# djeedai/bevy_hanabi

Measured on AMD Instinct MI355X. Metric: particle-updates/sec, higher is better.
Workload: dtype f32

## Files before the change

### bevy_hanabi_amd/csrc/hnb_kernels.hip.h

```cpp
#pragma once
#ifndef __HIPCC_RTC__
#include <hip/hip_runtime.h>
#endif
#include "hnb_dev.h"

namespace hnb {

template <class T>
__device__ __forceinline__ T* global_ptr(uint64_t addr) {
    typedef __attribute__((address_space(1))) T global_t;
    return (T*)(global_t*)addr;
}

struct u2_t { uint32_t x, y; };
struct u3_t { uint32_t x, y, z; };
typedef uint32_t u4v __attribute__((ext_vector_type(4)));
#if defined(HNB_NONTEMPORAL) || defined(HNB_NONTEMPORAL_LOADS)
#define HNB_NT_LOAD(p) __builtin_nontemporal_load(p)
#else
#define HNB_NT_LOAD(p) (*(p))
#endif
#if defined(HNB_NONTEMPORAL) || defined(HNB_NONTEMPORAL_STORES)
#define HNB_NT_STORE(v, p) __builtin_nontemporal_store(v, p)
#else
#define HNB_NT_STORE(v, p) (*(p) = (v))
#endif

template <class T> __device__ __forceinline__ T ld_hint(const T* p, bool nt) { return nt ? __builtin_nontemporal_load(p) : *p; }
template <class T> __device__ __forceinline__ void st_hint(T v, T* p, bool nt) { if (nt) __builtin_nontemporal_store(v, p); else *p = v; }

__device__ __forceinline__ void lds_barrier() { asm volatile("s_waitcnt lgkmcnt(0)\n\ts_barrier" ::: "memory"); }

#define HNB_DPP_(v, ident, ctrl, rows) ((uint32_t)__builtin_amdgcn_update_dpp((int)(ident), (int)(v), ctrl, rows, 0xf, false))
#define HNB_WAVE_STEP_(v, ident, OP, ctrl, rows) { const uint32_t t_ = HNB_DPP_(v, ident, ctrl, rows); v = OP(v, t_); }
#define HNB_WAVE_REDUCE_(v, ident, OP)                                                          \
    HNB_WAVE_STEP_(v, ident, OP, 0xB1, 0xf)                            \
    HNB_WAVE_STEP_(v, ident, OP, 0x4E, 0xf)                            \
    HNB_WAVE_STEP_(v, ident, OP, 0x124, 0xf)                                     \
    HNB_WAVE_STEP_(v, ident, OP, 0x128, 0xf)   \
    HNB_WAVE_STEP_(v, ident, OP, 0x142, 0xa)                \
    HNB_WAVE_STEP_(v, ident, OP, 0x143, 0xc)
__device__ __forceinline__ uint32_t wave_sum_u32(uint32_t v) {
#define HNB_OP_(a, b) ((a) + (b))
    HNB_WAVE_REDUCE_(v, 0u, HNB_OP_)
#undef HNB_OP_
    return (uint32_t)__builtin_amdgcn_readlane((int)v, 63);
}
__device__ __forceinline__ uint32_t wave_min_u32(uint32_t v) {
#define HNB_OP_(a, b) ((b) < (a) ? (b) : (a))
    HNB_WAVE_REDUCE_(v, 0xffffffffu, HNB_OP_)
#undef HNB_OP_
    return (uint32_t)__builtin_amdgcn_readlane((int)v, 63);
}
__device__ __forceinline__ uint32_t wave_max_u32(uint32_t v) {
#define HNB_OP_(a, b) ((b) > (a) ? (b) : (a))
    HNB_WAVE_REDUCE_(v, 0u, HNB_OP_)
#undef HNB_OP_
    return (uint32_t)__builtin_amdgcn_readlane((int)v, 63);
}
__device__ __forceinline__ float wave_min_f32(float x) {
    uint32_t v = f2u(x);
#define HNB_OP_(a, b) f2u(fminf(u2f(a), u2f(b)))
    HNB_WAVE_REDUCE_(v, 0x7f800000u, HNB_OP_)
#undef HNB_OP_
    return u2f((uint32_t)__builtin_amdgcn_readlane((int)v, 63));
}


#ifndef HNB_JIT_TU
__global__ void k_reset_lists(uint32_t* __restrict__ dead, uint32_t* __restrict__ alive0, uint32_t* __restrict__ alive1, uint32_t capacity) {
    uint32_t i = blockIdx.x * blockDim.x + threadIdx.x;
    if (i < capacity) { dead[i] = i; alive0[i] = 0u; alive1[i] = 0u; }
}
#endif

#ifndef HNB_JIT_TU
struct ProbeArgs { uint32_t n_planes; uint32_t stride16[8]; uint64_t off[8]; uint32_t write_mask; uint32_t salt; uint64_t n_quads; };
__global__ void __launch_bounds__(256) k_probe_placement(char* __restrict__ base, const ProbeArgs a) {
    const uint64_t q = (uint64_t)blockIdx.x * 256u + threadIdx.x;
    if (q >= a.n_quads) return;
    uint32_t acc = 0;
#pragma unroll
    for (uint32_t pl = 0; pl < 8; ++pl) {
        if (pl >= a.n_planes) break;
        uint4* ptr = reinterpret_cast<uint4*>(base + a.off[pl]) + q * a.stride16[pl];
        for (uint32_t i = 0; i < a.stride16[pl]; ++i) {
            uint4 v = ptr[i];
            acc += v.x + v.y + v.z + v.w;
            v.x ^= a.salt;
            if (a.write_mask >> pl & 1u) ptr[i] = v;
        }
    }
    if (acc == 0x9e3779b9u && a.salt) *reinterpret_cast<uint32_t*>(base) = acc;
}
#endif

template <class FILE_T>
__device__ __forceinline__ void vfile_store_attr(const FILE_T& r, uint32_t ncomp, uint32_t reg, char* plane, uint32_t slot) {
    switch (ncomp) {
        case 1: reinterpret_cast<uint32_t*>(plane)[slot] = r[reg]; break;
        case 2: reinterpret_cast<u2_t*>(plane)[slot] = u2_t{r[reg], r[reg + 1]}; break;
        case 3: reinterpret_cast<u3_t*>(plane)[slot] = u3_t{r[reg], r[reg + 1], r[reg + 2]}; break;
        default: reinterpret_cast<uint4*>(plane)[slot] = make_uint4(r[reg], r[reg + 1], r[reg + 2], r[reg + 3]); break;
    }
}
__device__ __forceinline__ Out4 vfile_load_attr(uint32_t ncomp, const char* plane, uint32_t slot) {
    Out4 o = Out4{0u, 0u, 0u, 0u};
    switch (ncomp) {
        case 1: o.v0 = reinterpret_cast<const uint32_t*>(plane)[slot]; break;
        case 2: { const u2_t t = reinterpret_cast<const u2_t*>(plane)[slot]; o.v0 = t.x; o.v1 = t.y; } break;
        case 3: { const u3_t t = reinterpret_cast<const u3_t*>(plane)[slot]; o.v0 = t.x; o.v1 = t.y; o.v2 = t.z; } break;
        default: { const uint4 t = reinterpret_cast<const uint4*>(plane)[slot]; o.v0 = t.x; o.v1 = t.y; o.v2 = t.z; o.v3 = t.w; } break;
    }
    return o;
}

__device__ __forceinline__ void pin_scalar(uint32_t v) { asm volatile("" ::"s"(v)); }
__device__ __forceinline__ uint32_t requested_spawn(const DevFrameInst& f) {
    const uint4 h0 = reinterpret_cast<const uint4*>(&f)[0], h1 = reinterpret_cast<const uint4*>(&f)[1];
    const uint32_t spawn_count = h0.x, parity = h1.z, skip = h1.w;
    const uint64_t ev_in = (uint64_t)h1.x | ((uint64_t)h1.y << 32);
    pin_scalar(spawn_count);
    if (skip) return 0u;
    if (ev_in == 0ull) return spawn_count;
    const DevEventBuffer* ev = global_ptr<const DevEventBuffer>(ev_in);
    const uint2 cnt = *reinterpret_cast<const uint2*>(ev->count);
    const uint32_t n = (parity ^ 1u) ? cnt.y : cnt.x, cap = ev->capacity;
    return n < cap ? n : cap;
}

struct InterpCode {
    using file_t = vreg_file_t;
    template <class ST>
    static __device__ __forceinline__ void run_init(const DevProgram& p, ST& S, const VmUniforms& U, const VmAttrIO& io) {
        vm_run<true, false>(p.init_code, p.init_len, S, U, nullptr, nullptr, io);
    }
    template <class ST>
    static __device__ __forceinline__ void run_update(const DevProgram& p, ST& S, const VmUniforms& U, const VmAttrIO& io) {
        vm_run<true, false>(p.update_code, p.update_len, S, U, nullptr, nullptr, io);
    }
    static __device__ __forceinline__ void zero_unassigned(const DevProgram& p, const VmAttrIO& io) {
        for (uint32_t a = 0; a < p.n_attrs; ++a) {
            if (p.attrs[a].reg != HNB_REG_NONE) continue;
            uint32_t* q = vm_attr_ptr(io, a);
            for (uint32_t c = 0; c < p.attrs[a].ncomp; ++c) q[c] = 0u;
        }
    }
    template <class ST>
    static __device__ __forceinline__ void store_init(const DevProgram& p, const ST& S, char* base, uint32_t slot) {
        for (uint32_t a = 0; a < p.n_attrs; ++a)
            if (p.attrs[a].reg != HNB_REG_NONE) vfile_store_attr(S.r, p.attrs[a].ncomp, p.attrs[a].reg, base + p.attrs[a].plane_off, slot);
    }
    template <class ST>
    static __device__ __forceinline__ void load_update(const DevProgram& p, ST& S, const char* base, uint32_t slot, bool valid) {
        for (uint32_t a = 0; a < p.n_attrs; ++a) {
            const DevAttr at = p.attrs[a];
            if (!(at.upd_flags & HNB_ATTR_UPD_LOAD) || at.reg == HNB_REG_NONE) continue;
            Out4 o = Out4{0u, 0u, 0u, 0u};
            if (valid) o = vfile_load_attr(at.ncomp, base + at.plane_off, slot);
            for (uint32_t cc = 0; cc < at.ncomp; ++cc) S.r[at.reg + cc] = out4_get(o, cc);
        }
    }
    template <class ST>
    static __device__ __forceinline__ void store_update(const DevProgram& p, const ST& S, char* base, uint32_t slot) {
// ... 867 lines not shown




__device__ __forceinline__ void store_died_bits(uint32_t* __restrict__ bits, uint32_t step_first, uint32_t nib, uint32_t lane) {
    int v = (int)(nib << (4u * (lane & 7u)));
    v |= __builtin_amdgcn_update_dpp(0, v, 0xB1, 0xf, 0xf, true);
    v |= __builtin_amdgcn_update_dpp(0, v, 0x4E, 0xf, 0xf, true);
    v |= __builtin_amdgcn_update_dpp(0, v, 0x141, 0xf, 0xf, true);
    if ((lane & 7u) == 0u) bits[(step_first >> 5) + (lane >> 3)] = (uint32_t)v;
}

struct StreamLds {
    uint32_t died[kBlock / 64];
    float lmin[kBlock / 64];
    uint32_t alive[kBlock / 64];
    float rem[kBlock / 64];
    uint32_t amin[kBlock / 64], amax[kBlock / 64];
    u4v xp[2][kBlock / 64][kStepRows * 3u / 4u];
};
__device__ __forceinline__ StreamLds& stream_lds() {
    __shared__ StreamLds s;
    return s;
}

template <class PROG, int PROBE, bool COHORT, bool FUSED = false>
__device__ __forceinline__ void update_stream_chunk(const SlotArgs& args, const uint64_t* __restrict__ inst_base, const DevFrameInst* __restrict__ fi,
                                                    const uint32_t* __restrict__ ublocks, const CompactBufs& cb,
                                                    const uint32_t wg, const uint32_t wg_total) {
    StreamLds& lds = stream_lds();
    uint32_t (&s_died)[kBlock / 64] = lds.died;
    float (&s_lmin)[kBlock / 64] = lds.lmin;
    uint32_t (&s_alive)[kBlock / 64] = lds.alive;
    float (&s_rem)[kBlock / 64] = lds.rem;
    uint32_t (&s_amin)[kBlock / 64] = lds.amin;
    uint32_t (&s_amax)[kBlock / 64] = lds.amax;
    u4v (&s_xp)[2][kBlock / 64][kStepRows * 3u / 4u] = lds.xp;
    const uint32_t tid = threadIdx.x, lane = tid & 63u, wave = tid >> 6;
    const bool split = !FUSED && !COHORT && args.quarters == 4u;
    const uint32_t S = FUSED ? args.fuse_steps : 1u;
    const uint32_t chunk = split ? chunk_of_workgroup(cb.xcd_remap, wg >> 2, wg_total >> 2) : chunk_of_workgroup(cb.xcd_remap, wg, wg_total);
    const uint32_t quarter = split ? (wg & 3u) : 0u;
    const uint32_t k = chunk / args.chunks_per_inst, j = chunk - k * args.chunks_per_inst;
    const uint32_t wave0 = j * kChunk + (split ? (quarter * (kBlock / 64u) + wave) * kStepRows : wave * kWaveRows);
    const uint32_t n_steps = split ? 1u : kWaveRows / kStepRows;
    const uint32_t n_words = split ? wg_total >> 2 : wg_total;
    const uint32_t frozen = fi[k].skip;
    const uint64_t slab = inst_base[k];
    const bool store_nt = args.store_hint != 0u;
#ifndef HNB_PUBLISH_FIRST_WG
#define HNB_PUBLISH_FIRST_WG 1
#endif
    if (args.safe_words && (HNB_PUBLISH_FIRST_WG ? wg == 0u : chunk == 0u)) {
        uint32_t* prev = args.safe_words + (size_t)(args.safe_parity ^ 1u) * args.safe_stride;
        uint32_t m = 0x7f800000u;
        for (uint32_t i = tid; i < n_words; i += kBlock) { const uint32_t v = prev[i]; prev[i] = 0x7f800000u; m = v < m ? v : m; }
        m = wave_min_u32(m);
        if (lane == 0) s_alive[wave] = m;
        __syncthreads();
        if (tid == 0u) {
            for (uint32_t w = 1; w < kBlock / 64; ++w) m = s_alive[w] < m ? s_alive[w] : m;
            *reinterpret_cast<volatile unsigned long long*>(args.safe_host) = ((unsigned long long)m << 32) | (unsigned long long)args.publish_tag;
        }
        __syncthreads();
    }
    if (args.skip_lists && j == 0u && quarter == 0u && tid == 0u) {
        DevMeta o = args.meta_in[k];
        if constexpr (FUSED) {
            DevMeta before = o;
            if (!frozen) {
                o.max_update = o.alive_count; o.dead_count = 0u; o.spawned = 0u; o.instance_count = o.alive_count;
                before = o;
                o.ref_write_index ^= S & 1u;
                before.ref_write_index ^= (S - 1u) & 1u;
            }
            DevMeta* row_in = const_cast<DevMeta*>(args.meta_in);
            ((S & 1u) ? args.meta_out : row_in)[k] = o;
            ((S & 1u) ? row_in : args.meta_out)[k] = before;
            cb.deaths[(size_t)(cb.parity ^ 1u) * cb.table_cap + k] = 0u;
        } else {
        if (!frozen) {
            o.ref_write_index ^= 1u;
            o.max_update = o.alive_count; o.dead_count = 0u; o.spawned = 0u; o.instance_count = o.alive_count;
        }
        args.meta_out[k] = o;
        cb.deaths[(size_t)(cb.parity ^ 1u) * cb.table_cap + k] = 0u;
        }
    }
    if (frozen) return;
    char* base = global_ptr<char>(slab);
    VmUniforms U;
    U.u = ublocks + (size_t)k * args.n_uregs * S;
    auto uniforms_of = [&](const uint32_t s) { VmUniforms Us = U; Us.u = U.u + (size_t)s * args.n_uregs; return Us; };
    U.xf = fi[k].xf;
    float rem_min = __builtin_inff();
    char* p_pos = base + args.plane_off[0];
    char* p_vel = base + args.plane_off[1];
    char* p_age = base + args.plane_off[2];
    char* p_life = base + args.plane_off[3];
    uint32_t* flags4 = reinterpret_cast<uint32_t*>(base + args.alive_flag_off);
    const uint32_t fl = args.flags;
    uint32_t died_total = 0;
    uint32_t* cfull = reinterpret_cast<uint32_t*>(base + args.lmin_off) + args.chunks_per_inst;
    const bool chunk_full = cfull[j] == 1u;
    uint32_t* astate = cfull + args.chunks_per_inst;
    uint32_t* aval = astate + args.chunks_per_inst;
    const uint32_t ast_raw = COHORT ? astate[j] : 0u;
    bool check_due = ((args.frame_phase + j) & 15u) == 0u;
    if constexpr (FUSED) {
        for (uint32_t s = 1; s < S; ++s) check_due = check_due || ((args.frame_phase + s + j) & 15u) == 0u;
    }
    const bool mixed = COHORT && ast_raw == 4u && !check_due;
    const uint32_t ast = ast_raw == 4u ? 0u : ast_raw;
    const float A = COHORT ? u2f(aval[j]) : 0.0f;
    uint32_t amin = 0xffffffffu, amax = 0u;
    uint32_t lane_alive = 0;
    const bool cull = args.cull_lifetime != 0u;
    float* lmin = reinterpret_cast<float*>(base + args.lmin_off);
    const float Lm = cull ? lmin[j] : 0.0f;
    const float dt_tick = cull ? uf(U, args.dt_operand) : 0.0f;
    auto age_after = [&](float a) {
        if constexpr (FUSED) {
            for (uint32_t s = 0; s < S; ++s) a = a + uf(uniforms_of(s), args.dt_operand);
            return a;
        } else return a + dt_tick;
    };
    if (args.horizon && j == 0u && quarter == 0u && tid == 0u) {
        double* clk = horizon_view(base, args.horizon_off, args.chunks_per_inst).clock;
        if constexpr (FUSED) {
            double c = *clk;
            for (uint32_t s = 0; s < S; ++s) { const float t = cull ? uf(uniforms_of(s), args.dt_operand) : 0.0f; c = c + (double)(t > 0.0f ? t : 0.0f) * (1.0 + 0x1p-16); }
            *clk = c;
        } else
        *clk = *clk + (double)(dt_tick > 0.0f ? dt_tick : 0.0f) * (1.0 + 0x1p-16);
    }
    float wave_min = __builtin_inff();
    bool loaded_all = true;
    bool flat = false;
    if constexpr (PROG::kFlat && COHORT && PROBE == 0) {
        flat = chunk_full && ast == 1u && cull && Lm > 0.0f && (age_after(A) < Lm) && (fl & 3u) == 3u && !(fl & 128u);
    }
    if (flat) {
        if constexpr (PROG::kFlat && COHORT && PROBE == 0) {
            const float A2 = age_after(A);
            u4v* pw = reinterpret_cast<u4v*>(p_pos + (size_t)j * (kChunk * 12u)) + wave * (kWaveRows * 3u / 4u);
            u4v* vw = reinterpret_cast<u4v*>(p_vel + (size_t)j * (kChunk * 12u)) + wave * (kWaveRows * 3u / 4u);
            const uint32_t rot = lane % 3u;
            if (args.age_current && (fl & 64u)) {
                u4v* aw = reinterpret_cast<u4v*>(p_age + (size_t)j * (kChunk * 4u)) + wave * (kWaveRows / 4u);
                const uint32_t a2 = f2u(A2);
#pragma unroll
                for (uint32_t step = 0; step < kWaveRows / kStepRows; ++step) aw[step * 64u + lane] = u4v{a2, a2, a2, a2};
            }
#pragma unroll 2
            for (uint32_t step = 0; step < kWaveRows / kStepRows; ++step) {
                float P[3][4], V[3][4];
#pragma unroll
                for (uint32_t w = 0; w < 3; ++w) {
                    const u4v a = pw[(step * 3u + w) * 64u + lane], b = vw[(step * 3u + w) * 64u + lane];
                    P[w][0] = u2f(a.x); P[w][1] = u2f(a.y); P[w][2] = u2f(a.z); P[w][3] = u2f(a.w);
                    V[w][0] = u2f(b.x); V[w][1] = u2f(b.y); V[w][2] = u2f(b.z); V[w][3] = u2f(b.w);
                }
                if constexpr (FUSED) {
                    for (uint32_t s = 0; s < S; ++s) PROG::run_flat(args.update_code, P, V, rot, uniforms_of(s));
                } else
                PROG::run_flat(args.update_code, P, V, rot, U);
#pragma unroll
                for (uint32_t w = 0; w < 3; ++w) {
                    if (fl & 16u) pw[(step * 3u + w) * 64u + lane] = u4v{f2u(P[w][0]), f2u(P[w][1]), f2u(P[w][2]), f2u(P[w][3])};
                    if (fl & 32u) vw[(step * 3u + w) * 64u + lane] = u4v{f2u(V[w][0]), f2u(V[w][1]), f2u(V[w][2]), f2u(V[w][3])};
                }
            }
            if (args.write_died && lane < kWaveRows / 32u)
                reinterpret_cast<uint32_t*>(base + args.died_bits_off)[((j * kChunk + wave * kWaveRows) >> 5) + lane] = 0u;
            amin = amax = f2u(A2);
            loaded_all = false;
            if (args.safe_words) rem_min = (f2u(A2) >> 31) ? 0.0f : (Lm - A2) - 1.0e-5f * Lm;
        }
    }
    auto step_body = [&](auto coh_tag, const uint32_t step, const uint32_t f4, const u4v* pre_age = nullptr) {
        constexpr bool COH = decltype(coh_tag)::value;
        const uint32_t s0 = wave0 + step * kStepRows + lane * 4u;
        bool was[4], fresh[4];
#pragma unroll
        for (int p = 0; p < 4; ++p) {
            const uint32_t byte = (f4 >> (8 * p)) & 0xffu;
            fresh[p] = COH && byte == 3u;
            was[p] = byte == 1u || fresh[p];
            lane_alive += was[p] ? 1u : 0u;
        }
        const bool any = was[0] || was[1] || was[2] || was[3];
        if (!__any(any)) {
            if (args.write_died) store_died_bits(reinterpret_cast<uint32_t*>(base + args.died_bits_off), s0 - lane * 4u, 0u, lane);
            return;
        }
        const bool full = was[0] && was[1] && was[2] && was[3];
        uint32_t slot[4];
#pragma unroll
        for (int p = 0; p < 4; ++p) slot[p] = s0 + p;
        bool lanes_on[4] = {any, any, any, any};
        Pinned<4> X;
#pragma unroll
        for (int p = 0; p < 4; ++p) { X.pos[p] = V3{0, 0, 0}; X.vel[p] = V3{0, 0, 0}; X.age[p] = 0.0f; X.lifetime[p] = 0.0f; X.alive[p] = true; }
        bool need_life = true;
        float age_was[4] = {0.0f, 0.0f, 0.0f, 0.0f};
        const uint32_t step_first = s0 - lane * 4u;
        const bool xp = args.transpose != 0u && PROBE == 0 && step_first + kStepRows <= args.capacity && __popcll(__ballot(any)) >= 32;
        if (xp) {
            if (fl & 1u) xpose_load3(X.pos, p_pos, step_first, s_xp[0][wave], lane);
            if (fl & 2u) xpose_load3(X.vel, p_vel, step_first, s_xp[1][wave], lane);
        }
        if (any) {
            if (!xp) {
                if (fl & 1u) pin_load3<4>(X.pos, p_pos, slot, lanes_on, true);
                if (fl & 2u) pin_load3<4>(X.vel, p_vel, slot, lanes_on, true);
            }
            if (fl & 4u) {
                if (!COH || ast != 1u) {
                    if (pre_age) { X.age[0] = u2f(pre_age->x); X.age[1] = u2f(pre_age->y); X.age[2] = u2f(pre_age->z); X.age[3] = u2f(pre_age->w); }
                    else pin_load1<4>(X.age, p_age, slot, lanes_on, true);
                    for (int p = 0; p < 4; ++p) age_was[p] = X.age[p];
                }
                if (COH && ast != 0u) {
#pragma unroll
                    for (int p = 0; p < 4; ++p) X.age[p] = fresh[p] ? X.age[p] : A;
                }
            }
        }
        if (cull && Lm > 0.0f && (COH || !mixed)) {
            bool may_die = false;
#pragma unroll
            for (int p = 0; p < 4; ++p) may_die = may_die || (was[p] && !(age_after(X.age[p]) < Lm));
            need_life = __any(may_die);
        }
        if (any && (fl & 8u)) {
            if (need_life) {
                if (args.stream_hint) {
                    const u4v ql = __builtin_nontemporal_load(reinterpret_cast<const u4v*>(p_life) + (slot[0] >> 2));
                    X.lifetime[0] = u2f(ql.x); X.lifetime[1] = u2f(ql.y); X.lifetime[2] = u2f(ql.z); X.lifetime[3] = u2f(ql.w);
                } else pin_load1<4>(X.lifetime, p_life, slot, lanes_on, true);
            }
            else {
#pragma unroll
                for (int p = 0; p < 4; ++p) X.lifetime[p] = Lm;
            }
        }
        if (!need_life) loaded_all = false;
        if constexpr (FUSED) {
            bool gone[4] = {false, false, false, false};
            for (uint32_t s = 0; s < S; ++s) {
                PROG::template run<4>(args.update_code, args.update_len, X, uniforms_of(s));
#pragma unroll
                for (int p = 0; p < 4; ++p) gone[p] = gone[p] || !X.alive[p];
            }
#pragma unroll
            for (int p = 0; p < 4; ++p) X.alive[p] = !gone[p];
        } else
        if constexpr (!(PROBE & 8)) PROG::template run<4>(args.update_code, args.update_len, X, U);
        if constexpr (!(PROBE & 4)) {
            const bool xp_pos = xp && (fl & 17u) == 17u, xp_vel = xp && (fl & 34u) == 34u;
            if (xp_pos) xpose_store3(X.pos, p_pos, step_first, s_xp[0][wave], lane, was, full, store_nt);
            if (xp_vel) xpose_store3(X.vel, p_vel, step_first, s_xp[1][wave], lane, was, full, store_nt);
            if (any) {
                if ((fl & 16u) && !xp_pos) pin_store3<4>(X.pos, p_pos, slot, was, full);
                if ((fl & 32u) && !xp_vel) pin_store3<4>(X.vel, p_vel, slot, was, full);
                if (fl & 64u) {
                    const bool plane_loaded = !COH || ast != 1u;
                    if (plane_loaded || args.age_current) {
                        if (plane_loaded && (fl & 4u) && !full) {
                            float q[4];
#pragma unroll
                            for (int p = 0; p < 4; ++p) q[p] = was[p] ? X.age[p] : age_was[p];
                            pin_store1<4>(q, p_age, slot, was, true, store_nt);
                        } else pin_store1<4>(X.age, p_age, slot, was, full, store_nt);
                    }
                }
                if (fl & 128u) pin_store1<4>(X.lifetime, p_life, slot, was, full);
            }
        } else {
            float acc = 0.0f;
#pragma unroll
            for (int p = 0; p < 4; ++p) acc += X.pos[p].x + X.pos[p].y + X.pos[p].z + X.vel[p].x + X.vel[p].y + X.vel[p].z + X.age[p] + X.lifetime[p];
            if (acc == 123.456f) X.alive[0] = false;
        }
        if (cull && need_life) {
#pragma unroll
            for (int p = 0; p < 4; ++p)
                if (was[p] && X.alive[p]) wave_min = fminf(wave_min, X.lifetime[p]);
        }
        if (args.safe_words) {
#pragma unroll
            for (int p = 0; p < 4; ++p)
                if (was[p] && X.alive[p]) rem_min = fminf(rem_min, (f2u(X.age[p]) >> 31) ? 0.0f : (X.lifetime[p] - X.age[p]) - 1.0e-5f * X.lifetime[p]);
        }
        if constexpr (COH) {
#pragma unroll
            for (int p = 0; p < 4; ++p) {
                const bool stays = was[p] && X.alive[p];
                const uint32_t b = f2u(X.age[p]);
                amin = (stays && b < amin) ? b : amin;
                amax = (stays && b > amax) ? b : amax;
            }
            if constexpr (!(PROBE & 4)) {
                const bool dies = (was[0] && !X.alive[0]) || (was[1] && !X.alive[1]) || (was[2] && !X.alive[2]) || (was[3] && !X.alive[3]);
                if (ast == 1u && (fl & 64u) && !args.age_current && __any(dies)) {
#pragma unroll
                    for (int p = 0; p < 4; ++p)
                        if (was[p] && !X.alive[p]) reinterpret_cast<float*>(p_age)[slot[p]] = X.age[p];
                }
            }
        }
        uint32_t nf = f4, nib = 0u;
        uint32_t died_here = 0;
#pragma unroll
        for (int p = 0; p < 4; ++p) {
            const bool died = was[p] && !X.alive[p];
            if (died) { nf &= ~(0xffu << (8 * p)); nib |= 1u << p; }
            else if (COH && fresh[p]) nf = (nf & ~(0xffu << (8 * p))) | (1u << (8 * p));
            died_here += (uint32_t)__popcll(__ballot(died));
        }
        if (nf != f4) flags4[s0 >> 2] = nf;
        if (args.write_died) store_died_bits(reinterpret_cast<uint32_t*>(base + args.died_bits_off), step_first, nib, lane);
        died_total += died_here;
    };
    if (!flat) {
// ... 540 lines not shown
```

### bevy_hanabi_amd/csrc/hnb_vm.h

```cpp
#pragma once
#include "hnb_math.h"
#ifdef __HIPCC_RTC__
#include "hanabi_amd.h"
#else
#include "../../include/hanabi_amd.h"
#endif

namespace hnb {

struct __attribute__((aligned(8))) Ins { uint32_t x, y; };

#ifdef HNB_VM_BOUNDS_CHECK
extern "C" void hnb_vm_oob(uint32_t index, uint32_t size);
template <uint32_t N>
struct checked_file_t {
    uint32_t v[N];
    uint32_t& operator[](uint32_t i) { if (i >= N) hnb_vm_oob(i, N); return v[i < N ? i : 0]; }
    const uint32_t& operator[](uint32_t i) const { if (i >= N) hnb_vm_oob(i, N); return v[i < N ? i : 0]; }
};
typedef checked_file_t<HNB_VM_MAX_REGS> vreg_file_t;
typedef checked_file_t<HNB_VM_MAX_REGS_WIDE> vreg_file_wide_t;
typedef checked_file_t<HNB_VM_MAX_UREGS> UFile;
#else
typedef uint32_t vreg_file_t __attribute__((vector_size(HNB_VM_MAX_REGS * 4)));
// ... 660 lines not shown
                const V3 v = uf3(U, a);
#pragma unroll
                for (int p = 0; p < P; ++p) mac_vel_add(X.vel[p], v);
            } break;
            case HNB_OP_M_PIN_SET: {
                if (d == HNB_REG_POSITION || d == HNB_REG_VELOCITY) {
                    const V3 v = uf3(U, a);
#pragma unroll
                    for (int p = 0; p < P; ++p) { if (d == HNB_REG_POSITION) X.pos[p] = v; else X.vel[p] = v; }
                } else {
                    const float s = uf(U, a);
#pragma unroll
                    for (int p = 0; p < P; ++p) { if (d == HNB_REG_AGE) X.age[p] = s; else X.lifetime[p] = s; }
                }
            } break;
            case HNB_OP_M_RADIAL_ACCEL:
                if constexpr (FULL) {
                    const V3 origin = uf3(U, a);
                    const float s = uf(U, b);
#pragma unroll
                    for (int p = 0; p < P; ++p) mac_radial_accel(X.pos[p], X.vel[p], origin, s);
                }
                break;
            case HNB_OP_M_TANGENT_ACCEL:
                if constexpr (FULL) {
                    const V3 origin = uf3(U, a), axis = uf3(U, b);
                    const float s = uf(U, c);
#pragma unroll
                    for (int p = 0; p < P; ++p) mac_tangent_accel(X.pos[p], X.vel[p], origin, axis, s);
                }
                break;
            case HNB_OP_M_CONFORM_SPHERE:
                if constexpr (FULL) {
                    ConformParams q;
                    q.c = uf3(U, a);
                    q.radius = uf(U, a + 3); q.influence_dist = uf(U, a + 4); q.shell_half_thickness = uf(U, a + 5);
                    q.max_attraction_speed = uf(U, a + 6); q.attraction_accel = uf(U, a + 7); q.sticky_factor = uf(U, a + 8);
                    const float dt = uf(U, b);
#pragma unroll
                    for (int p = 0; p < P; ++p) mac_conform_sphere(X.pos[p], X.vel[p], q, dt);
                }
                break;
            case HNB_OP_M_KILL_SPHERE: {
                const V3 center = uf3(U, a);
                const float r2 = uf(U, b);
#pragma unroll
                for (int p = 0; p < P; ++p) mac_kill_sphere(X.pos[p], center, r2, (aux & 1u) != 0u, X.alive[p]);
            } break;
            case HNB_OP_M_KILL_AABB: {
                const V3 center = uf3(U, a), half = uf3(U, b);
#pragma unroll
                for (int p = 0; p < P; ++p) mac_kill_aabb(X.pos[p], center, half, (aux & 1u) != 0u, X.alive[p]);
            } break;
            default: break;
        }
    }
}


template <uint32_t OP, int P>
HNB_HD void apply_static(const Ins ins, Pinned<P>& X, const VmUniforms& U) {
    const uint32_t a = HNB_OPERAND_DECODE((ins.x >> 16) & 0xffu, ins.y >> 13), b = HNB_OPERAND_DECODE(ins.x >> 24, ins.y >> 14);
    const uint32_t c = HNB_OPERAND_DECODE(ins.y & 0xffu, ins.y >> 15), aux = ins.y >> 16;
    if constexpr (OP == HNB_OP_M_AGE_TICK) {
        const float dt = uf(U, a);
        const bool has_lifetime = (aux & 1u) != 0u;
#pragma unroll
        for (int p = 0; p < P; ++p) mac_age_tick(X.age[p], X.lifetime[p], dt, has_lifetime, X.alive[p]);
    } else if constexpr (OP == HNB_OP_M_EULER) {
        const float dt = uf(U, a);
#pragma unroll
        for (int p = 0; p < P; ++p) mac_euler(X.pos[p], X.vel[p], dt);
    } else if constexpr (OP == HNB_OP_M_VEL_SCALE) {
        const float s = uf(U, a);
#pragma unroll
        for (int p = 0; p < P; ++p) mac_vel_scale(X.vel[p], s);
    } else if constexpr (OP == HNB_OP_M_VEL_ADD) {
        const V3 v = uf3(U, a);
#pragma unroll
        for (int p = 0; p < P; ++p) mac_vel_add(X.vel[p], v);
    } else if constexpr (OP == HNB_OP_M_PIN_SET) {
        const uint32_t d = (ins.x >> 8) & 0xffu;
        if (d == HNB_REG_POSITION || d == HNB_REG_VELOCITY) {
            const V3 v = uf3(U, a);
#pragma unroll
            for (int p = 0; p < P; ++p) { if (d == HNB_REG_POSITION) X.pos[p] = v; else X.vel[p] = v; }
        } else {
            const float s = uf(U, a);
#pragma unroll
            for (int p = 0; p < P; ++p) { if (d == HNB_REG_AGE) X.age[p] = s; else X.lifetime[p] = s; }
        }
    } else if constexpr (OP == HNB_OP_M_RADIAL_ACCEL) {
        const V3 origin = uf3(U, a);
        const float s = uf(U, b);
#pragma unroll
        for (int p = 0; p < P; ++p) mac_radial_accel(X.pos[p], X.vel[p], origin, s);
    } else if constexpr (OP == HNB_OP_M_TANGENT_ACCEL) {
        const V3 origin = uf3(U, a), axis = uf3(U, b);
        const float s = uf(U, c);
#pragma unroll
        for (int p = 0; p < P; ++p) mac_tangent_accel(X.pos[p], X.vel[p], origin, axis, s);
    } else if constexpr (OP == HNB_OP_M_CONFORM_SPHERE) {
        ConformParams q;
        q.c = uf3(U, a);
        q.radius = uf(U, a + 3); q.influence_dist = uf(U, a + 4); q.shell_half_thickness = uf(U, a + 5);
        q.max_attraction_speed = uf(U, a + 6); q.attraction_accel = uf(U, a + 7); q.sticky_factor = uf(U, a + 8);
        const float dt = uf(U, b);
#pragma unroll
        for (int p = 0; p < P; ++p) mac_conform_sphere(X.pos[p], X.vel[p], q, dt);
    } else if constexpr (OP == HNB_OP_M_KILL_SPHERE) {
        const V3 center = uf3(U, a);
        const float r2 = uf(U, b);
        const bool inside = (aux & 1u) != 0u;
#pragma unroll
        for (int p = 0; p < P; ++p) mac_kill_sphere(X.pos[p], center, r2, inside, X.alive[p]);
    } else if constexpr (OP == HNB_OP_M_KILL_AABB) {
        const V3 center = uf3(U, a), half = uf3(U, b);
        const bool inside = (aux & 1u) != 0u;
#pragma unroll
        for (int p = 0; p < P; ++p) mac_kill_aabb(X.pos[p], center, half, inside, X.alive[p]);
    } else {
        static_assert(OP == HNB_OP_M_AGE_TICK, "apply_static: opcode is not a streamable macro op");
    }
}

HNB_HD float rot3(const V3 v, uint32_t c) { return c == 0u ? v.x : (c == 1u ? v.y : v.z); }
template <uint32_t OP>
HNB_HD void apply_static_flat(const Ins ins, float (&pos)[3][4], float (&vel)[3][4], uint32_t rot, const VmUniforms& U) {
    const uint32_t a = HNB_OPERAND_DECODE((ins.x >> 16) & 0xffu, ins.y >> 13);
    if constexpr (OP == HNB_OP_M_EULER) {
        const float dt = uf(U, a);
#pragma unroll
        for (int j = 0; j < 3; ++j)
#pragma unroll
            for (int e = 0; e < 4; ++e) pos[j][e] = pos[j][e] + vel[j][e] * dt;
    } else if constexpr (OP == HNB_OP_M_VEL_SCALE) {
        const float s = uf(U, a);
#pragma unroll
        for (int j = 0; j < 3; ++j)
#pragma unroll
            for (int e = 0; e < 4; ++e) vel[j][e] = vel[j][e] * s;
    } else if constexpr (OP == HNB_OP_M_VEL_ADD) {
        const V3 v = uf3(U, a);
        const float vr[3] = {rot3(v, rot % 3u), rot3(v, (rot + 1u) % 3u), rot3(v, (rot + 2u) % 3u)};
#pragma unroll
        for (int j = 0; j < 3; ++j)
#pragma unroll
            for (int e = 0; e < 4; ++e) vel[j][e] = vel[j][e] + vr[(j + e) % 3];
    } else {
        static_assert(OP == HNB_OP_M_AGE_TICK, "apply_static_flat: not a component-wise op");
    }
}

struct ProgInterp {
    static constexpr bool kFlat = false;
    static constexpr bool kAgeOnly = false;
    HNB_HD_MEMBER static void run_flat(const Ins* __restrict__, float (&)[3][4], float (&)[3][4], uint32_t, const VmUniforms&) {}
    static constexpr uint32_t kLen = 0;
    template <int P> HNB_HD_MEMBER static void run(const Ins* __restrict__ code, uint32_t n_ins, Pinned<P>& X, const VmUniforms& U) {
        fast_run<P, true>(code, n_ins, X, U);
    }
};
struct ProgNone {
    static constexpr bool kFlat = false;
    static constexpr bool kAgeOnly = false;
    HNB_HD_MEMBER static void run_flat(const Ins* __restrict__, float (&)[3][4], float (&)[3][4], uint32_t, const VmUniforms&) {}
    static constexpr uint32_t kLen = 0;
    template <int P> HNB_HD_MEMBER static void run(const Ins* __restrict__, uint32_t, Pinned<P>&, const VmUniforms&) {}
    static bool matches(const Ins*, uint32_t n_ins) { return n_ins == 0; }
};
template <uint32_t... OPS>
struct ProgStatic {
    static constexpr uint32_t kLen = sizeof...(OPS);
    static constexpr bool kFlat = ((OPS == HNB_OP_M_AGE_TICK || OPS == HNB_OP_M_EULER || OPS == HNB_OP_M_VEL_SCALE || OPS == HNB_OP_M_VEL_ADD) && ...) &&
                                  ((OPS == HNB_OP_M_AGE_TICK) || ...);
    static constexpr bool kAgeOnly = sizeof...(OPS) > 0 && ((OPS == HNB_OP_M_AGE_TICK) && ...);
    HNB_HD_MEMBER static void run_flat(const Ins* __restrict__ code, float (&pos)[3][4], float (&vel)[3][4], uint32_t rot, const VmUniforms& U) {
        if constexpr (kFlat) {
            uint32_t i = 0;
            ((apply_static_flat<OPS>(code[i++], pos, vel, rot, U)), ...);
        }
    }
    template <int P> HNB_HD_MEMBER static void run(const Ins* __restrict__ code, uint32_t, Pinned<P>& X, const VmUniforms& U) {
        uint32_t i = 0;
        ((apply_static<OPS, P>(code[i++], X, U)), ...);
    }
    static bool matches(const Ins* code, uint32_t n_ins) {
        const uint32_t ops[] = {OPS...};
        if (n_ins != kLen) return false;
        for (uint32_t i = 0; i < kLen; ++i)
            if ((code[i].x & 0xffu) != ops[i]) return false;
        return true;
    }
};

}
```

Baseline: 126.3 billion.

## Hoist flat-op uniforms to scalar loads and double-buffer the flat step loop

In the flat cohort path, operand decoding and uniform fetches are now resolved once per wave through constant-address-space (scalar) loads into a small FlatOp array. The per-step loop no longer re-reads the instruction stream and uniforms for every step. The non-fused loop is software-pipelined with double-buffered position and velocity registers, fully unrolled so the next step's loads are issued before the current step computes. A specialised variant removes the per-store flag checks when both position and velocity are written. This trades higher register pressure, which could reduce occupancy, for better latency hiding and less redundant scalar work.

Measured after the change: 126.6 billion, median of 6. About the same (+0.2%).

```diff
diff --git a/bevy_hanabi_amd/csrc/hnb_kernels.hip.h b/bevy_hanabi_amd/csrc/hnb_kernels.hip.h
--- a/bevy_hanabi_amd/csrc/hnb_kernels.hip.h
+++ b/bevy_hanabi_amd/csrc/hnb_kernels.hip.h
@@ -10,6 +10,11 @@
 __device__ __forceinline__ T* global_ptr(uint64_t addr) {
     typedef __attribute__((address_space(1))) T global_t;
     return (T*)(global_t*)addr;
+}
+
+__device__ __forceinline__ uint32_t ld_const_u32(const uint32_t* p) {
+    typedef __attribute__((address_space(4))) const uint32_t const_t;
+    return *(const_t*)(uint64_t)p;
 }
 
 struct u2_t { uint32_t x, y; };
@@ -1183,25 +1188,52 @@
 #pragma unroll
                 for (uint32_t step = 0; step < kWaveRows / kStepRows; ++step) aw[step * 64u + lane] = u4v{a2, a2, a2, a2};
             }
-#pragma unroll 2
-            for (uint32_t step = 0; step < kWaveRows / kStepRows; ++step) {
-                float P[3][4], V[3][4];
+            constexpr uint32_t kOps = PROG::kFlatOps;
+            const uint32_t* code_w = reinterpret_cast<const uint32_t*>(args.update_code);
+            uint32_t opnd[kOps];
+#pragma unroll
+            for (uint32_t i = 0; i < kOps; ++i) opnd[i] = i < PROG::kLen ? flat_operand_of(ld_const_u32(code_w + 2u * i), ld_const_u32(code_w + 2u * i + 1u)) : 0u;
+            FlatOp R[kOps];
+            if constexpr (!FUSED) PROG::resolve_flat(opnd, [&](const uint32_t r) { return ld_const_u32(U.u + r); }, R);
+            auto run = [&](float (&P)[3][4], float (&V)[3][4]) {
+                if constexpr (FUSED) {
+                    for (uint32_t s = 0; s < S; ++s) {
+                        const uint32_t* us = U.u + (size_t)s * args.n_uregs;
+                        FlatOp Rs[kOps];
+                        PROG::resolve_flat(opnd, [&](const uint32_t r) { return ld_const_u32(us + r); }, Rs);
+                        PROG::run_flat(Rs, P, V, rot);
+                    }
+                } else PROG::run_flat(R, P, V, rot);
+            };
+            auto load = [&](const uint32_t step, float (&P)[3][4], float (&V)[3][4]) {
 #pragma unroll
                 for (uint32_t w = 0; w < 3; ++w) {
                     const u4v a = pw[(step * 3u + w) * 64u + lane], b = vw[(step * 3u + w) * 64u + lane];
                     P[w][0] = u2f(a.x); P[w][1] = u2f(a.y); P[w][2] = u2f(a.z); P[w][3] = u2f(a.w);
                     V[w][0] = u2f(b.x); V[w][1] = u2f(b.y); V[w][2] = u2f(b.z); V[w][3] = u2f(b.w);
                 }
-                if constexpr (FUSED) {
-                    for (uint32_t s = 0; s < S; ++s) PROG::run_flat(args.update_code, P, V, rot, uniforms_of(s));
-                } else
-                PROG::run_flat(args.update_code, P, V, rot, U);
-#pragma unroll
-                for (uint32_t w = 0; w < 3; ++w) {
-                    if (fl & 16u) pw[(step * 3u + w) * 64u + lane] = u4v{f2u(P[w][0]), f2u(P[w][1]), f2u(P[w][2]), f2u(P[w][3])};
-                    if (fl & 32u) vw[(step * 3u + w) * 64u + lane] = u4v{f2u(V[w][0]), f2u(V[w][1]), f2u(V[w][2]), f2u(V[w][3])};
+            };
+            auto walk = [&](auto both_tag) {
+                constexpr bool BOTH = decltype(both_tag)::value;
+                constexpr uint32_t kSteps = kWaveRows / kStepRows;
+                constexpr bool PIPE = !FUSED;
+                constexpr uint32_t kUnroll = PIPE ? kSteps : 2u;
+                float P[2][3][4], V[2][3][4];
+                if constexpr (PIPE) load(0u, P[0], V[0]);
+#pragma unroll kUnroll
+                for (uint32_t step = 0; step < kSteps; ++step) {
+                    const uint32_t c = PIPE ? step & 1u : 0u;
+                    if constexpr (PIPE) { if (step + 1u < kSteps) load(step + 1u, P[c ^ 1u], V[c ^ 1u]); }
+                    else load(step, P[c], V[c]);
+                    run(P[c], V[c]);
+#pragma unroll
+                    for (uint32_t w = 0; w < 3; ++w) {
+                        if (BOTH || (fl & 16u)) pw[(step * 3u + w) * 64u + lane] = u4v{f2u(P[c][w][0]), f2u(P[c][w][1]), f2u(P[c][w][2]), f2u(P[c][w][3])};
+                        if (BOTH || (fl & 32u)) vw[(step * 3u + w) * 64u + lane] = u4v{f2u(V[c][w][0]), f2u(V[c][w][1]), f2u(V[c][w][2]), f2u(V[c][w][3])};
+                    }
                 }
-            }
+            };
+            if ((fl & 48u) == 48u) walk(BoolTag<true>{}); else walk(BoolTag<false>{});
             if (args.write_died && lane < kWaveRows / 32u)
                 reinterpret_cast<uint32_t*>(base + args.died_bits_off)[((j * kChunk + wave * kWaveRows) >> 5) + lane] = 0u;
             amin = amax = f2u(A2);
diff --git a/bevy_hanabi_amd/csrc/hnb_vm.h b/bevy_hanabi_amd/csrc/hnb_vm.h
--- a/bevy_hanabi_amd/csrc/hnb_vm.h
+++ b/bevy_hanabi_amd/csrc/hnb_vm.h
@@ -836,6 +836,40 @@
     }
 }
 
+struct FlatOp { float x, y, z; };
+HNB_HD uint32_t flat_operand_of(const uint32_t ins_x, const uint32_t ins_y) { return HNB_OPERAND_DECODE((ins_x >> 16) & 0xffu, ins_y >> 13) & 0xffu; }
+template <uint32_t OP, class LOADU>
+HNB_HD void resolve_static_flat(const uint32_t a, LOADU&& load_u, FlatOp& o) {
+    o.x = (OP == HNB_OP_M_AGE_TICK) ? 0.0f : u2f(load_u(a));
+    o.y = o.z = 0.0f;
+    if constexpr (OP == HNB_OP_M_VEL_ADD) { o.y = u2f(load_u(a + 1u)); o.z = u2f(load_u(a + 2u)); }
+}
+template <uint32_t OP>
+HNB_HD void apply_resolved_flat(const FlatOp& o, float (&pos)[3][4], float (&vel)[3][4], uint32_t rot) {
+    if constexpr (OP == HNB_OP_M_EULER) {
+        const float dt = o.x;
+#pragma unroll
+        for (int j = 0; j < 3; ++j)
+#pragma unroll
+            for (int e = 0; e < 4; ++e) pos[j][e] = pos[j][e] + vel[j][e] * dt;
+    } else if constexpr (OP == HNB_OP_M_VEL_SCALE) {
+        const float s = o.x;
+#pragma unroll
+        for (int j = 0; j < 3; ++j)
+#pragma unroll
+            for (int e = 0; e < 4; ++e) vel[j][e] = vel[j][e] * s;
+    } else if constexpr (OP == HNB_OP_M_VEL_ADD) {
+        const V3 v = V3{o.x, o.y, o.z};
+        const float vr[3] = {rot3(v, rot % 3u), rot3(v, (rot + 1u) % 3u), rot3(v, (rot + 2u) % 3u)};
+#pragma unroll
+        for (int j = 0; j < 3; ++j)
+#pragma unroll
+            for (int e = 0; e < 4; ++e) vel[j][e] = vel[j][e] + vr[(j + e) % 3];
+    } else {
+        static_assert(OP == HNB_OP_M_AGE_TICK, "apply_resolved_flat: not a component-wise op");
+    }
+}
+
 struct ProgInterp {
     static constexpr bool kFlat = false;
     static constexpr bool kAgeOnly = false;
@@ -865,6 +899,20 @@
             ((apply_static_flat<OPS>(code[i++], pos, vel, rot, U)), ...);
         }
     }
+    static constexpr uint32_t kFlatOps = kLen ? kLen : 1u;
+    template <class LOADU>
+    HNB_HD_MEMBER static void resolve_flat(const uint32_t (&opnd)[kFlatOps], LOADU&& load_u, FlatOp (&R)[kFlatOps]) {
+        if constexpr (kFlat) {
+            uint32_t i = 0;
+            ((resolve_static_flat<OPS>(opnd[i], load_u, R[i]), ++i), ...);
+        }
+    }
+    HNB_HD_MEMBER static void run_flat(const FlatOp (&R)[kFlatOps], float (&pos)[3][4], float (&vel)[3][4], uint32_t rot) {
+        if constexpr (kFlat) {
+            uint32_t i = 0;
+            ((apply_resolved_flat<OPS>(R[i++], pos, vel, rot)), ...);
+        }
+    }
     template <int P> HNB_HD_MEMBER static void run(const Ins* __restrict__ code, uint32_t, Pinned<P>& X, const VmUniforms& U) {
         uint32_t i = 0;
         ((apply_static<OPS, P>(code[i++], X, U)), ...);
```
